# pvphan/camera-calibration

Hardware: AMD Instinct MI355X
Metric: LM iters/sec & residuals/sec, 10k-view checkerboard @1/2/4/8 GPU (higher is better)
Workload: dtype f64

## Files before the change

camera-calibration_amd/calibrate.py:

```python
import operator
import time

import numpy as np

from . import distortion
from . import engine
from . import fixed as fixedmod
from . import jacobian
from . import mathutils as mu
from . import uncertainty as uncertaintymod


class Calibrator:
    _λinitial = engine.LAMBDA_INITIAL
    _λmin = engine.LAMBDA_MIN
    _λmax = engine.LAMBDA_MAX
    _Pt_error_min = engine.PT_ERROR_MIN

    def __init__(self, distortionModel: distortion.DistortionModel, *, fixed=(), dtype="f64", device=0):
        self._distortionModel = distortionModel
        self.setFixed(fixed)
        self._jac = None
        self._dtype = dtype
        self._device = device
# ... 16 lines not shown
            return P0
        return fixedmod.applyFixedValues(P0, self._fixedValues)

    def calibrate(self, allDetections, maxIters):
        Ainitial, Winitial, kInitial = self.estimateCalibrationParameters(allDetections)
        return self.refineCalibrationParameters(Ainitial, Winitial, kInitial, allDetections,
                                                maxIters, shouldPrint=True)

    def calibrateExtended(self, allDetections, maxIters):
        sse, A, W, k = self.calibrate(allDetections, maxIters)
        return sse, A, W, k, self.uncertainty(A, W, k, allDetections)

    def uncertainty(self, A, W, k, allDetections):
        P = self._composeParameterVector(A, W, k).ravel()
        eng = self._resident.getFromDetections(allDetections)
        eng.setFixedShared(self._fixedMask)
        cov = eng.covariance(P, wantViews=True, wantCross=False)
        errs = eng.viewErrors(P)
        return uncertaintymod.fromEngineResults(self._distortionModel.sharedParameterNames(), cov, errs, eng.MN,
                                                values=P, fixedMask=self._fixedMask)

    def estimateCalibrationParameters(self, allDetections):
        from . import linearcalibrate
        offs, sensor, model = engine.packDetections(allDetections)
        A, W, k = linearcalibrate.estimateCalibrationParametersDevice(self._distortionModel, offs, sensor, model,
                                                                      self._device)
        return A, list(W), k

    def _refineHomographies(self, Hs, allDetections):
        offs, sensor, model = engine.packDetections(allDetections)
        return list(engine.refineHomographies(Hs, offs, sensor, model, 20, self._device))

    def _refineHomography(self, H, sensorPoints, modelPoints, jac=None):
        s = np.asarray(sensorPoints, dtype=np.float64).reshape(-1, 2)
        m = np.asarray(modelPoints, dtype=np.float64).reshape(-1, 3)
        offs = np.array([0, s.shape[0]], dtype=np.int64)
        return engine.refineHomographies(np.asarray(H, dtype=np.float64).reshape(1, 3, 3), offs, s, m, 20,
                                         self._device)[0]

    def _projectPointsHomography(self, H, modelPoints):
        modelPoints = np.asarray(modelPoints, dtype=np.float64)
        return mu.unhom((np.asarray(H, dtype=np.float64) @ mu.hom(modelPoints[:, :2]).T).T)

    def refineCalibrationParameters(self, Ainitial, Winitial, kInitial, allDetections,
                                    maxIters, shouldPrint=False):
        self._initializeJacobian()
        if not isinstance(self._jac, jacobian.ProjectionJacobian):
            raise TypeError(f"Calibrator._jac was replaced by {type(self._jac).__name__}: the device refinement "
                            "evaluates the closed-form projection Jacobian inside its kernels and cannot consult an "
                            "injected Jacobian object; use jacobian.ProjectionJacobian (or leave _jac unset)")
        maxIters = operator.index(maxIters)
        if maxIters <= 0:
            raise UnboundLocalError("local variable 'Pt_error' referenced before assignment")
        t0 = time.perf_counter()
        Pt = self._composeParameterVector(Ainitial, Winitial, kInitial)
        t1 = time.perf_counter()
        eng = self._resident.getFromDetections(allDetections)
        sse, P, iters, trace = self._refineOn(eng, Pt, maxIters, shouldPrint)
        t3 = time.perf_counter()
        Arefined, Wrefined, kRefined = self._decomposeParameterVector(P)
        self.lastSeconds.update(compose=t1 - t0, decompose=time.perf_counter() - t3)
        return sse, Arefined, Wrefined, kRefined

    def refinePacked(self, P0, viewOffsets, sensorPoints, modelPoints, maxIters, shouldPrint=False, sameProblem=False):
        if maxIters <= 0:
            raise UnboundLocalError("local variable 'Pt_error' referenced before assignment")
        eng = self._resident.get(viewOffsets, sensorPoints, modelPoints, sameProblem=sameProblem)
        return self._refineOn(eng, P0, maxIters, shouldPrint)

    def _refineOn(self, eng, P0, maxIters, shouldPrint):
        t0 = time.perf_counter()
        eng.setFixedShared(self._fixedMask)
        P0 = self._startPoint(P0)
        if not shouldPrint:
            out = eng.refine(P0, maxIters, self._λinitial, self._λmin, self._λmax, self._Pt_error_min)
        else:
            out = self._refineVerbose(eng, P0, maxIters)
        self.lastSeconds = dict(self._resident.lastSeconds, lm=time.perf_counter() - t0, iters=int(out[2]))
        self.lastTrace = out[3]
        return out

    def _refineVerbose(self, eng, P0, maxIters):
        ts = time.time()
        eng.lmBegin(P0, maxIters, self._λinitial, self._λmin, self._λmax, self._Pt_error_min)
        eng.lmRun(1)
        for it in range(maxIters):
            eng.lmRun(1)
            row, itersDone = eng.peekTrace(it)
            if itersDone > it:
                error = row[1] if not (row[2] < row[1]) else row[2]
                self._printIterationStats(it, ts, row[5:], error, row[3])
            if eng.lmDone():
                break
        return eng.lmEnd()

    def refinePoses(self, A, Winitial, k, allDetections, maxIters):
        modelId = self._distortionModel.modelId
        L = engine.NUM_SHARED[modelId]
        P = engine.composeParameters(modelId, A, Winitial, k, self._device)
        offs, sensor, model = engine.packDetections(allDetections)
        sse, poses, iters, status = engine.refinePoses(modelId, P[:L], P[L:].reshape(-1, 6), offs, sensor, model,
                                                       operator.index(maxIters), self._λinitial, self._λmin, self._λmax,
                                                       self._Pt_error_min, self._device)
        _, W, _ = engine.decomposeParameters(modelId, np.concatenate((P[:L], poses.ravel())), self._device)
        return sse, list(W), iters, status

    def estimatePoses(self, A, k, allDetections, maxIters=20):
        offs, sensor, model = engine.packDetections(allDetections)
        Hs = engine.estimateHomographies(offs, sensor, model, 20, self._device)
        Winitial = engine.computeExtrinsics(Hs, A, self._device)
        return self.refinePoses(A, Winitial, k, allDetections, maxIters)

    def _initializeJacobian(self):
        if self._jac is None:
            self._jac = jacobian.ProjectionJacobian(self._distortionModel, self._dtype, self._device)
# ... 34 lines not shown
```

camera-calibration_amd/csrc/calib_lm.hip:

```cpp
#include "../../include/calib_lm.h"
#include "kernels.hpp"
#include "host_rows.hpp"
#include "launch_plan.hpp"
#include "shard_layout.hpp"

#include <hip/hip_runtime.h>
#include <hip/hip_ext.h>
#include <algorithm>
#include <atomic>
#include <cmath>
#include <cstdio>
#include <cstdlib>
#include <dlfcn.h>
#include <chrono>
#include <future>
#include <memory>
#include <mutex>
#include <thread>
#include <cstring>
#include <new>
#include <string>
#include <type_traits>
#include <vector>

// ... 76 lines not shown
        return r.empty() ? "none" : r;
    }
    int model = 0, dtype = 0, device = 0;
    int L = 10, C = 16;
    hipStream_t own_stream = nullptr;
    hipStream_t stream = nullptr;

    bool has_problem = false;
    int64_t M = 0, MN = 0;
    int nv = 0;
    int n_items = 0;
    int64_t n_tiles = 0;
    int max_views_per_tile = 1;
    int uniform_n = 0;
    Knobs knobs;
    LaunchPlan plan;
    std::vector<ShardChunk> chunks;
    int64_t max_chunk_points = 0;
    DevBuf<unsigned char> uv, XY, Z, VC, J, r, y;
    template <typename U> static U* as(const DevBuf<unsigned char>& b) { return reinterpret_cast<U*>(b.p); }
    template <typename U> U* uv_as() const { return as<U>(uv); }
    template <typename U> U* XY_as() const { return as<U>(XY); }
    template <typename U> U* Z_as() const { return as<U>(Z); }
    template <typename U> U* VC_as() const { return as<U>(VC); }
    template <typename U> U* J_as() const { return as<U>(J); }
    template <typename U> U* r_as() const { return as<U>(r); }
    template <typename U> U* y_as() const { return as<U>(y); }
    DevBuf<int> pt_view, view_ext, item_n, view_item0, item_view;
    DevBuf<uint32_t> emit_tab;
    DevBuf<int32_t> stream_ops;
    int lm_mode = CALIB_LM_FUSED;
    uint32_t fixed_mask = 0;
    int num_cus = 256;
    DevBuf<int64_t> item_pt0;
    DevBuf<double> sse_part, G[2], bpart, part, red_own, P[2], Peval, trace;
    int n_bpart = 0;
    DevBuf<LMState> st, st_eval;
    double* red = nullptr;
    void* comm = nullptr;
    DevBuf<double> rccl_test;
    int comm_ranks = 0, comm_rank = 0;
    void* peer_mem = nullptr;
    std::vector<void*> peer_open;
    DevBuf<unsigned long long*> peer_slots;
    std::vector<unsigned long long*> peer_slot_host;
    DevBuf<int> peer_flags;
    int peer_world = 0, peer_rank = 0;
    unsigned peer_epoch = 0;
    double peer_timeout_s = 60.0;
    bool peer_connected = false;
    bool exchange_round = false;
    int* host_done = nullptr;
    int* host_done_dev = nullptr;
    bool lm_active = false;
    int lm_max_iters = 0;
    int rounds_enqueued = 0;

    bool cov_pending = false;
    std::vector<int64_t> ext_offsets;
    bool ext_offsets_on_device = false;
    DevBuf<int64_t> ext_offsets_dev;
    DevBuf<double> view_err, cov_css, cov_views, cov_cross;
    DevBuf<int> cov_flag;

    bool stage_ready = false;
    void* stage_pinned = nullptr;
    hipStream_t stage_stream[4] = {nullptr, nullptr, nullptr, nullptr};
    void* stage_buf[4][2] = {{nullptr, nullptr}, {nullptr, nullptr}, {nullptr, nullptr}, {nullptr, nullptr}};
    hipEvent_t stage_ev[4][2] = {{nullptr, nullptr}, {nullptr, nullptr}, {nullptr, nullptr}, {nullptr, nullptr}};

    bool prof = false;
    int prof_stride = 1;
    int64_t prof_seen[3] = {0, 0, 0};
    std::vector<hipEvent_t> ev;
    std::vector<int> ev_kind;
    size_t ev_used = 0;
};

namespace {

size_t tsize(const calib_handle_s* h) { return h->dtype == CALIB_DTYPE_F64 ? 8 : 4; }

int prof_reserve(calib_handle_s* h, int kind) {
    if (!h->prof || h->ev_used + 2 > h->ev.size()) return -1;
    if (h->prof_seen[kind]++ % h->prof_stride != 0) return -1;
    int idx = (int)h->ev_used;
    h->ev_used += 2;
    h->ev_kind[idx / 2] = kind;
    return idx;
}

template <typename F, typename... Args>
void launch_kind(calib_handle_s* h, int kind, F kernel, dim3 grid, dim3 block, size_t shmem, Args... args) {
    const int idx = prof_reserve(h, kind);
    if (idx >= 0)
        hipExtLaunchKernelGGL(kernel, grid, block, (uint32_t)shmem, h->stream, h->ev[(size_t)idx], h->ev[(size_t)idx + 1], 0, args...);
    else
        hipLaunchKernelGGL(kernel, grid, block, shmem, h->stream, args...);
}

calib_handle_s* const kNoHandle = nullptr;

static_assert(CALIB_MODEL_RADTAN == kRadtan && CALIB_MODEL_FISHEYE == kFisheye, "the C ABI's model ids are the kernels'");
template <int MODEL_, typename T_>
struct Form {
    static constexpr int MODEL = MODEL_, L = ModelTraits<MODEL_>::L, C = ModelTraits<MODEL_>::C;
// ... 396 lines not shown
        if (rc) return rc;
    }
    if (MN > 0) {
        const int rc = pack_points(h, lay, sensor_uv, model_xyz, lap);
        if (rc) return rc;
    }
    h->has_problem = true;
    return CALIB_OK;
}

struct LocalSlots { hipIpcMemHandle_t ipc; void* mem; int device; };
std::vector<LocalSlots> g_local_slots;
std::mutex g_local_slots_mutex;

void peer_release(calib_handle_s* h) {
    for (void* m : h->peer_open)
        if (m) (void)hipIpcCloseMemHandle(m);
    h->peer_open.clear();
    if (h->peer_mem) {
        std::lock_guard<std::mutex> lock(g_local_slots_mutex);
        for (size_t i = 0; i < g_local_slots.size(); ++i)
            if (g_local_slots[i].mem == h->peer_mem) { g_local_slots.erase(g_local_slots.begin() + (long)i); break; }
    }
    if (h->peer_mem) (void)hipFree(h->peer_mem);
    h->peer_mem = nullptr;
    h->peer_slots.release();
    h->peer_slot_host.clear();
    h->peer_flags.release();
    h->peer_connected = false;
    h->peer_world = 0;
}

int peer_fault_check(calib_handle_s* h) {
    if (!h->peer_connected) return CALIB_OK;
    int fault = 0;
    HIP_TRY(hipMemcpy(&fault, h->peer_flags.p, sizeof(int), hipMemcpyDeviceToHost));
    if (fault)
        return fail(CALIB_E_HIP, "peer exchange: a rank's contribution did not arrive before the deadline "
                                 "(the ranks no longer run in lockstep, or a peer died)");
    return CALIB_OK;
}

int lm_finish(calib_handle_s* h, LMState* s) {
    SYNC_H(h);
    HIP_TRY(hipMemcpy(s, st_cur(h), sizeof(*s), hipMemcpyDeviceToHost));
    h->lm_active = false;
    const int prc = peer_fault_check(h);
    if (prc) return prc;
    if (s->error == CALIB_E_SINGULAR)
        return fail(CALIB_E_SINGULAR, "Singular matrix: damped normal equations are not invertible");
    return CALIB_OK;
}

int lm_run(calib_handle_t h, int rounds, int check_every, bool sharded) {
    CHECK_H(h);
    if (!h->lm_active) return fail(CALIB_E_STATE, "calib_lm_begin has not been called");
    const bool peers = sharded && h->peer_connected;
    for (int i = 0; i < rounds; ++i) {
        h->exchange_round = peers;
        int rc = calib_lm_local(h);
        h->exchange_round = false;
        if (rc) return rc;
        if (sharded && !peers) {
            rc = calib_lm_allreduce(h);
            if (rc) return rc;
        }
        rc = calib_lm_update(h);
        if (rc) return rc;
        if (peers && h->host_done && *static_cast<volatile int*>(h->host_done) == 2)
            return fail(CALIB_E_HIP, "peer exchange: a rank's contribution did not arrive before the deadline "
                                     "(the ranks no longer run in lockstep, or a peer died); no further rounds are enqueued");
        if (check_every > 0 && !sharded && h->host_done) {
            if (*static_cast<volatile int*>(h->host_done)) break;
        } else if (check_every > 0 && (i + 1) % check_every == 0 && i + 1 < rounds) {
            int done = 0;
            rc = calib_lm_done(h, &done);
            if (rc) return rc;
            if (done) break;
        }
    }
    return CALIB_OK;
}

int check_views(int64_t num_views, const int64_t* view_offsets, const double* sensor_uv, const double* model_xyz) {
    if (num_views < 0 || !view_offsets) return fail(CALIB_E_INVALID, "null argument");
    if (num_views == 0) return CALIB_OK;
    const int64_t MN = view_offsets[num_views];
    if (view_offsets[0] != 0 || MN < 0 || (MN > 0 && (!sensor_uv || !model_xyz)))
        return fail(CALIB_E_INVALID, "bad view_offsets / point arrays");
    for (int64_t i = 0; i < num_views; ++i)
        if (view_offsets[i + 1] < view_offsets[i]) return fail(CALIB_E_INVALID, "view_offsets must be non-decreasing");
    return CALIB_OK;
}

int use_device(int device_id) {
    int ndev = 0;
    HIP_TRY(hipGetDeviceCount(&ndev));
    if (device_id < 0 || device_id >= ndev) return fail(CALIB_E_HIP, "no such HIP device (no CPU fallback)");
    HIP_TRY(hipSetDevice(device_id));
    return CALIB_OK;
}

int homography_pipeline(int64_t num_views, const int64_t* view_offsets, const double* sensor_uv,
                        const double* model_xyz, double* H, bool dlt, int refine_iters, int device_id) {
    if (!H) return fail(CALIB_E_INVALID, "null argument");
    int rc = check_views(num_views, view_offsets, sensor_uv, model_xyz);
    if (rc || num_views == 0) return rc;
    rc = use_device(device_id);
    if (rc) return rc;
    const int64_t MN = view_offsets[num_views];
    std::vector<double> xy((size_t)MN * 2);
    for (int64_t p = 0; p < MN; ++p) { xy[2 * p] = model_xyz[3 * p]; xy[2 * p + 1] = model_xyz[3 * p + 1]; }
    DevBuf<int64_t> doffs;
    DevBuf<double2> duv, dxy;
    DevBuf<double> dH;
    HIP_TRY(doffs.alloc((size_t)num_views + 1));
    HIP_TRY(duv.alloc((size_t)std::max<int64_t>(MN, 1)));
    HIP_TRY(dxy.alloc((size_t)std::max<int64_t>(MN, 1)));
    HIP_TRY(dH.alloc((size_t)num_views * 9));
    HIP_TRY(hipMemcpy(doffs.p, view_offsets, ((size_t)num_views + 1) * 8, hipMemcpyHostToDevice));
    if (MN) HIP_TRY(hipMemcpy(duv.p, sensor_uv, (size_t)MN * 16, hipMemcpyHostToDevice));
    if (MN) HIP_TRY(hipMemcpy(dxy.p, xy.data(), (size_t)MN * 16, hipMemcpyHostToDevice));
    if (!dlt) HIP_TRY(hipMemcpy(dH.p, H, (size_t)num_views * 72, hipMemcpyHostToDevice));
    const unsigned blocks = (unsigned)((num_views + 15) / 16);
    if (dlt) {
        hipLaunchKernelGGL(dlt_kernel, dim3(blocks), dim3(256), 0, 0, doffs.p, (const double2*)duv.p, (const double2*)dxy.p,
                           num_views, dH.p);
// ... 233 lines not shown

    auto fetch2 = [&](const void* dev, double* out) -> int {
        if (h->dtype == CALIB_DTYPE_F64) {
            HIP_TRY(hipMemcpy(out, dev, (size_t)MN * 16, hipMemcpyDeviceToHost));
        } else {
            std::vector<float> tmp((size_t)MN * 2);
            HIP_TRY(hipMemcpy(tmp.data(), dev, tmp.size() * 4, hipMemcpyDeviceToHost));
            for (size_t i = 0; i < tmp.size(); ++i) out[i] = tmp[i];
        }
        return CALIB_OK;
    };
    if (out_y && MN) { rc = fetch2(h->y.p, out_y); if (rc) return rc; }
    if (out_r && MN) { rc = fetch2(h->r.p, out_r); if (rc) return rc; }
    if (out_Jc && MN) {
        const int C = h->C;
        const size_t cnt = MN4 * C * 2;
        std::vector<double> tmp(cnt);
        if (h->dtype == CALIB_DTYPE_F64) {
            HIP_TRY(hipMemcpy(tmp.data(), h->J.p, cnt * 8, hipMemcpyDeviceToHost));
        } else {
            std::vector<float> tf(cnt);
            HIP_TRY(hipMemcpy(tf.data(), h->J.p, cnt * 4, hipMemcpyDeviceToHost));
            for (size_t i = 0; i < cnt; ++i) tmp[i] = tf[i];
        }
        for (int64_t p = 0; p < MN; ++p)
            for (int c = 0; c < C; ++c) {
                out_Jc[(p * 2 + 0) * C + c] = tmp[(size_t)jIndex(p, c, C) * 2 + 0];
                out_Jc[(p * 2 + 1) * C + c] = tmp[(size_t)jIndex(p, c, C) * 2 + 1];
            }
    }
    return CALIB_OK;
}

int calib_lm_reduce_size(calib_handle_t h, int64_t* out_num_doubles) {
    if (!h || !out_num_doubles) return fail(CALIB_E_INVALID, "null argument");
    *out_num_doubles = reduceSize(h->L);
    return CALIB_OK;
}

int calib_lm_bind_reduce_buffer(calib_handle_t h, void* reduce_dev) {
    CHECK_H(h);
    SYNC_H(h);
    HIP_TRY(h->red_own.alloc((size_t)reduceSize(h->L)));
    h->red = reduce_dev ? reinterpret_cast<double*>(reduce_dev) : h->red_own.p;
    return CALIB_OK;
}

int calib_lm_begin(calib_handle_t h, const double* P0, int max_iters, double lam_init, double lam_min,
                   double lam_max, double err_min) {
    CHECK_H(h);
    int rc = need_problem(h);
    if (rc) return rc;
    if (!P0) return fail(CALIB_E_INVALID, "P0 is null");
    h->cov_pending = false;
    if (max_iters <= 0)
        return fail(CALIB_E_INVALID, "max_iters must be >= 1 (the reference raises UnboundLocalError "
                                     "for maxIters=0, src/calibrate.py:171)");
    if (h->nv != h->M)
        return fail(CALIB_E_SINGULAR, "a view without points makes J^T J + lambda diag(J^T J) singular");
    const size_t ts = tsize(h);
    const int64_t K = numParams(h);
    if (h->lm_mode == CALIB_LM_TWO_KERNEL)
        HIP_TRY(h->J.alloc((size_t)((h->max_chunk_points + 3) / 4 * 4) * h->C * 2 * ts));
    for (int b = 0; b < 2; ++b) {
        const bool fresh = !h->G[b].p || h->G[b].n < (size_t)num_records(h) * kGStride;
        HIP_TRY(h->G[b].alloc((size_t)num_records(h) * kGStride));
        if (fresh) HIP_TRY(hipMemsetAsync(h->G[b].p, 0, h->G[b].n * 8, h->stream));
    }
    HIP_TRY(h->bpart.alloc(((size_t)std::max(h->n_items, 1) + h->chunks.size()) * kPartStride));
    HIP_TRY(h->part.alloc((size_t)2 * h->plan.schur_blocks * variantSize(h->L)));
    HIP_TRY(h->red_own.alloc((size_t)reduceSize(h->L)));
    if (!h->red) h->red = h->red_own.p;
    HIP_TRY(h->P[0].alloc((size_t)K));
    HIP_TRY(h->P[1].alloc((size_t)K));
    HIP_TRY(h->st.alloc(2));
    HIP_TRY(h->trace.alloc((size_t)max_iters * (CALIB_TRACE_HEADER + h->L)));
    HIP_TRY(hipMemsetAsync(h->trace.p, 0, (size_t)max_iters * (CALIB_TRACE_HEADER + h->L) * 8, h->stream));
    HIP_TRY(hipMemcpyAsync(h->P[0].p, P0, (size_t)K * 8, hipMemcpyHostToDevice, h->stream));
    HIP_TRY(hipMemcpyAsync(h->P[1].p, P0, (size_t)K * 8, hipMemcpyHostToDevice, h->stream));
    LMState s;
    std::memset(&s, 0, sizeof(s));
    s.lam = lam_init; s.lam_min = lam_min; s.lam_max = lam_max; s.err_min = err_min;
    if (!h->host_done) {
        void* p = nullptr;
        if (hipHostMalloc(&p, sizeof(int), hipHostMallocMapped) == hipSuccess) h->host_done = static_cast<int*>(p);
        else (void)hipGetLastError();
        void* dp = nullptr;
        if (h->host_done && hipHostGetDevicePointer(&dp, h->host_done, 0) == hipSuccess) h->host_done_dev = static_cast<int*>(dp);
        else (void)hipGetLastError();
    }
    if (h->host_done) {
        if (h->lm_active) SYNC_H(h);
        *h->host_done = 0;
        s.notify = h->host_done_dev;
    }
    s.cur = 1;
    s.fixed_mask = (int)h->fixed_mask;
    s.max_iters = max_iters;
    HIP_TRY(hipMemsetAsync(h->st.p, 0, 2 * sizeof(LMState), h->stream));
    HIP_TRY(hipMemcpyAsync(h->st.p, &s, sizeof(s), hipMemcpyHostToDevice, h->stream));
    SYNC_H(h);
    h->lm_active = true;
    h->lm_max_iters = max_iters;
    h->rounds_enqueued = 0;
    return CALIB_OK;
}

int calib_lm_local(calib_handle_t h) {
    CHECK_H(h);
    if (!h->lm_active) return fail(CALIB_E_STATE, "calib_lm_begin has not been called");
    LMState* st = st_cur(h);
    int rc = CALIB_OK;
    if (h->rounds_enqueued == 0) {
        rc = launch_view_setup(h, h->P[0].p, h->P[1].p, st, 1);
        if (rc) return rc;
    }
    if (h->lm_mode == CALIB_LM_FUSED) {
        rc = launch_fused(h, st, 1);
        if (rc) return rc;
        return launch_schur_reduce(h, st, h->red);
    }
    h->n_bpart = 0;
    for (const auto& c : h->chunks) {
        rc = launch_jacobian(h, h->P[0].p, h->P[1].p, st, 1, true, true, false, false, c.p0, c.p1);
        if (rc) return rc;
        rc = launch_gram(h, st, 1, c.item0, c.item1, c.p0);
        if (rc) return rc;
    }
    return launch_schur_reduce(h, st, h->red);
}

int calib_lm_update(calib_handle_t h) {
    CHECK_H(h);
    if (!h->lm_active) return fail(CALIB_E_STATE, "calib_lm_begin has not been called");
    const int rc = launch_update_backsub(h);
    h->rounds_enqueued += 1;
    return rc;
}

int calib_lm_done(calib_handle_t h, int* out_done) {
    CHECK_H(h);
    if (!h->lm_active || !out_done) return fail(CALIB_E_STATE, "no LM run active");
    LMState s;
    HIP_TRY(hipMemcpyAsync(&s, st_cur(h), sizeof(s), hipMemcpyDeviceToHost, h->stream));
    SYNC_H(h);
    *out_done = s.done;
    return peer_fault_check(h);
}

int calib_lm_peek_trace(calib_handle_t h, int iter, double* out_row, int* out_iters) {
    CHECK_H(h);
    if (!h->lm_active || !out_row || !out_iters) return fail(CALIB_E_STATE, "no LM run active");
    if (iter < 0 || iter >= h->lm_max_iters) return fail(CALIB_E_INVALID, "trace row out of range");
    LMState s;
    const size_t w = (size_t)(CALIB_TRACE_HEADER + h->L);
    HIP_TRY(hipMemcpyAsync(&s, st_cur(h), sizeof(s), hipMemcpyDeviceToHost, h->stream));
    HIP_TRY(hipMemcpyAsync(out_row, h->trace.p + (size_t)iter * w, w * 8, hipMemcpyDeviceToHost, h->stream));
    SYNC_H(h);
// ... 516 lines not shown
    return CALIB_OK;
}

int calib_compose_params(int model, int64_t num_views, const double* A, const double* W, const double* k,
                         double* P_out, int device_id) {
    if (!known_model(model)) return fail(CALIB_E_INVALID, "unknown distortion model");
    if (num_views < 0 || !A || !k || !P_out || (num_views > 0 && !W)) return fail(CALIB_E_INVALID, "null argument");
    const int nk = num_distortion(model), L = 5 + nk;
    P_out[0] = A[0]; P_out[1] = A[4]; P_out[2] = A[1]; P_out[3] = A[2]; P_out[4] = A[5];
    for (int j = 0; j < nk; ++j) P_out[5 + j] = k[j];
    if (num_views == 0) return CALIB_OK;
    int rc = use_device(device_id);
    if (rc) return rc;
    DevBuf<double> dW, dP;
    HIP_TRY(dW.alloc((size_t)num_views * 16));
    HIP_TRY(dP.alloc((size_t)L + 6 * (size_t)num_views));
    HIP_TRY(hipMemcpy(dW.p, W, (size_t)num_views * 128, hipMemcpyHostToDevice));
    hipLaunchKernelGGL(compose_views_kernel, dim3((unsigned)((num_views + 255) / 256)), dim3(256), 0, 0, dW.p, num_views, L, dP.p);
    LAUNCHED(kNoHandle, "compose_views_kernel");
    HIP_TRY(hipMemcpy(P_out + L, dP.p + L, (size_t)num_views * 48, hipMemcpyDeviceToHost));
    return CALIB_OK;
}

int calib_decompose_params(int model, int64_t num_views, const double* P, double* A_out, double* W_out,
                           double* k_out, int device_id) {
    if (!known_model(model)) return fail(CALIB_E_INVALID, "unknown distortion model");
    if (num_views < 0 || !P || (num_views > 0 && !W_out)) return fail(CALIB_E_INVALID, "null argument");
    const int nk = num_distortion(model), L = 5 + nk;
    if (A_out) {
        const double a[9] = {P[0], P[2], P[3], 0.0, P[1], P[4], 0.0, 0.0, 1.0};
        std::memcpy(A_out, a, sizeof(a));
    }
    if (k_out) for (int j = 0; j < nk; ++j) k_out[j] = P[5 + j];
    if (num_views == 0) return CALIB_OK;
    int rc = use_device(device_id);
    if (rc) return rc;
    DevBuf<double> dW, dP;
    HIP_TRY(dW.alloc((size_t)num_views * 16));
    HIP_TRY(dP.alloc((size_t)L + 6 * (size_t)num_views));
    HIP_TRY(hipMemcpy(dP.p, P, ((size_t)L + 6 * (size_t)num_views) * 8, hipMemcpyHostToDevice));
    hipLaunchKernelGGL(decompose_views_kernel, dim3((unsigned)((num_views + 255) / 256)), dim3(256), 0, 0, dP.p, num_views, L, dW.p);
    LAUNCHED(kNoHandle, "decompose_views_kernel");
    HIP_TRY(hipMemcpy(W_out, dW.p, (size_t)num_views * 128, hipMemcpyDeviceToHost));
    return CALIB_OK;
}

int calib_refine_awk(calib_handle_t h, double* A_inout, double* W_inout, double* k_inout, int max_iters,
                     double lam_init, double lam_min, double lam_max, double err_min, double* out_sse,
                     int* out_iters, double* out_trace) {
    CHECK_H(h);
    int rc = need_problem(h);
    if (rc) return rc;
    if (!A_inout || !k_inout || (h->M > 0 && !W_inout)) return fail(CALIB_E_INVALID, "null argument");
    std::vector<double> P((size_t)numParams(h));
    rc = calib_compose_params(h->model, h->M, A_inout, W_inout, k_inout, P.data(), h->device);
    if (rc) return rc;
    rc = calib_refine(h, P.data(), max_iters, lam_init, lam_min, lam_max, err_min, out_sse, out_iters, out_trace);
    if (rc) return rc;
    return calib_decompose_params(h->model, h->M, P.data(), A_inout, W_inout, k_inout, h->device);
}

int calib_profile_enable(calib_handle_t h, int on) {
    CHECK_H(h);
    SYNC_H(h);
    if (on && h->ev.empty()) {
        h->ev.resize(kEventPool);
        h->ev_kind.assign(kEventPool / 2, 0);
        for (auto& e : h->ev) HIP_TRY(hipEventCreate(&e));
    }
    h->prof = on != 0;
    h->prof_stride = on > 1 ? on : 1;
    h->prof_seen[0] = h->prof_seen[1] = h->prof_seen[2] = 0;
    h->ev_used = 0;
    return CALIB_OK;
}

int calib_profile_read(calib_handle_t h, int which, double* out_total_ms, int64_t* out_launches) {
    CHECK_H(h);
    if (!out_total_ms || !out_launches) return fail(CALIB_E_INVALID, "null argument");
    SYNC_H(h);
    double total = 0.0;
    int64_t count = 0;
    for (size_t i = 0; i + 1 < h->ev_used; i += 2) {
        if (h->ev_kind[i / 2] != which) continue;
        float ms = 0.f;
        HIP_TRY(hipEventElapsedTime(&ms, h->ev[i], h->ev[i + 1]));
        total += ms;
        count += 1;
    }
    *out_total_ms = total;
    *out_launches = count;
    return CALIB_OK;
}

int calib_view_errors(calib_handle_t h, const double* P, double* out_view_sse, double* out_view_rms,
                      double* out_view_max) {
    CHECK_H(h);
    int rc = need_problem(h);
    if (rc) return rc;
    if (!P) return fail(CALIB_E_INVALID, "P is null");
    if (h->lm_active)
        return fail(CALIB_E_STATE, "a stepping LM run is active on this handle (calib_lm_end it first)");
    const int64_t M = h->M;
    if (M == 0) return CALIB_OK;
    if (!h->ext_offsets_on_device) {
        HIP_TRY(h->ext_offsets_dev.alloc((size_t)M + 1));
        HIP_TRY(hipMemcpy(h->ext_offsets_dev.p, h->ext_offsets.data(), ((size_t)M + 1) * 8, hipMemcpyHostToDevice));
        h->ext_offsets_on_device = true;
    }
    HIP_TRY(h->view_err.alloc((size_t)M * 3));
    HIP_TRY(hipMemcpyAsync(h->Peval.p, P, (size_t)numParams(h) * 8, hipMemcpyHostToDevice, h->stream));
    rc = launch_view_setup(h, h->Peval.p, nullptr, h->st_eval.p, 0);
// ... 108 lines not shown
```

camera-calibration_amd/csrc/kernels.hpp:

```cpp
#pragma once
#include "point_model.hpp"
#include <stdint.h>
#include <type_traits>

namespace calib {

constexpr int kTile = 256;
constexpr int kGramChunk = 512;
constexpr int kGramUnroll = 4;
constexpr int kGRows = 0;
constexpr int kGStride = 96;
__host__ __device__ __forceinline__ constexpr int gvSlot(int L, int j) { return j < 5 ? L + 1 + j : 16 + L + 2; }
__host__ __device__ __forceinline__ constexpr int gvOfSlot(int L, int slot) {
    const int m = slot >> 4, n = (slot & 15) - L;
    return (m == 0 && n >= 1 && n <= 5) ? n - 1 : ((m == 1 && n == 2) ? 5 : -1);
}
constexpr int kPartStride = 112;
constexpr int kMaxL = 10;

constexpr int kEmitZero = 256;
constexpr int kEmitTile = 264;
constexpr int kEmitTabSize = kGStride + kPartStride;
inline void buildEmitTable(int C, uint32_t* tab ) {
    const int L = C - 6;
// ... 1490 lines not shown
    const double gci = useB ? gS : gA;
#pragma unroll
    for (int j = 0; j < L; ++j) {
        brow[j] = useB ? bS[j] : bA[j];
        row[j] = brow[j] - (useB ? sB[j] : sA[j]);
    }
    row[L] = gci - (useB ? rhsB : rhsA);
#pragma unroll
    for (int j = 0; j < L; ++j) if (j == i) row[j] += lam * brow[j];
    const int fixed_mask = in->fixed_mask;
    const bool fixed_i = (fixed_mask >> i) & 1;
    if (fixed_mask != 0) {
#pragma unroll
        for (int j = 0; j < L; ++j) {
            const bool fixed_j = (fixed_mask >> j) & 1;
            row[j] = (fixed_i || fixed_j) ? (j == i ? 1.0 : 0.0) : row[j];
        }
        row[L] = fixed_i ? 0.0 : row[L];
    }
    if (!done) {
        double saved[L + 1];
#pragma unroll
        for (int j = 0; j <= L; ++j) saved[j] = row[j];
        if (!spd_solve_wave0<L>(row, i, dc)) {
            int myCol = -1;
            double d = 0.0;
            if (gauss_jordan16<L, true>(saved, i, myCol, d)) { error = -3; done = true; }
#pragma unroll
            for (int c = 0; c < L; ++c) dc[c] = group_sum16(myCol == c ? d : 0.0);
        }
    } else {
#pragma unroll
        for (int c = 0; c < L; ++c) dc[c] = 0.0;
    }

    if (writer) {
        if (i < L) {
#pragma unroll
            for (int j = 0; j < L; ++j) out->B[i * L + j] = brow[j];
            out->gc[i] = gci;
            double dci = 0.0;
#pragma unroll
            for (int c = 0; c < L; ++c) if (c == i) dci = dc[c];
            out->dc[i] = dci;
            if (!done) Pb[cur ^ 1][i] = fixed_i ? Pb[cur][i] : Pb[cur][i] + dci;
        }
        if (w0) {
            out->lam = lam; out->err_cur = err_cur_new; out->last_err = last_err;
            out->lam_min = in->lam_min; out->lam_max = in->lam_max; out->err_min = in->err_min;
            out->cur = cur; out->round = round + 1; out->iters = iters; out->max_iters = in->max_iters;
            out->done = done ? 1 : 0; out->error = error; out->accepted_last = accepted; out->fixed_mask = fixed_mask;
            out->notify = in->notify;
            if (done && in->notify) __hip_atomic_store(in->notify, 1, __ATOMIC_RELAXED, __HIP_MEMORY_SCOPE_SYSTEM);
        }
    }
    cur_out = cur;
    lam_out = lam;
    return !done;
}

template <int L, typename T>
__device__ __forceinline__ void finish_view(const double (&V)[21], const double (&invd)[6], const double (&z)[6],
                                            double coef, int c, int v, const int* __restrict__ view_ext,
                                            const double* __restrict__ Pc, double* __restrict__ Pn,
                                            T* __restrict__ VC) {
    double w[6];
#pragma unroll
    for (int m = 0; m < 6; ++m) w[m] = group_sum16(coef * z[m]);
    double d[6];
    backward6(V, invd, w, d);
    const int64_t o = L + 6 * (int64_t)view_ext[v];
    double en[6];
#pragma unroll
    for (int m = 0; m < 6; ++m) en[m] = Pc[o + m] + d[m];
    if (c < 6) {
        double ev = en[0];
#pragma unroll
        for (int m = 1; m < 6; ++m) ev = (c == m) ? en[m] : ev;
        Pn[o + c] = ev;
    }
    const double deg = 0.017453292519943295;
    double sn[3], cs[3];
    {
        const int a = c & 3;
        const double th = (a == 1 ? en[1] : (a == 2 ? en[2] : en[0])) * deg;
        double s1, c1;
        sincos(th, &s1, &c1);
        if (fabs(th) <= 1e-8) { s1 = 0.0; c1 = 1.0; }
        sn[0] = quad_bcast<0>(s1); sn[1] = quad_bcast<1>(s1); sn[2] = quad_bcast<2>(s1);
        cs[0] = quad_bcast<0>(c1); cs[1] = quad_bcast<1>(c1); cs[2] = quad_bcast<2>(c1);
    }
    const double sx = sn[0], cx = cs[0], sy = sn[1], cy = cs[1], sz = sn[2], cz = cs[2];
    const double o18[18] = {cz * cy, cz * sy * sx - sz * cx, cz * sy * cx + sz * sx,
                            sz * cy, sz * sy * sx + cz * cx, sz * sy * cx - cz * sx,
                            -sy, cy * sx, cy * cx, en[3], en[4], en[5],
                            deg * cz * cy, deg * sz * cy, -deg * sy, -deg * sz, deg * cz, 0.0};
    double mine = o18[0];
#pragma unroll
    for (int j = 1; j < 16; ++j) mine = (c == j) ? o18[j] : mine;
    T* dst = VC + (int64_t)v * kViewStride;
    dst[c] = (T)mine;
    if (c < 2) dst[16 + c] = (T)(c == 0 ? o18[16] : o18[17]);
}

template <typename T>
struct UpdArgs {
// ... 781 lines not shown
```

camera-calibration_amd/csrc/launch_plan.hpp:

```cpp
#pragma once
#include "../../include/calib_lm.h"
#include "kernels.hpp"

#include <algorithm>
#include <cstdint>
#include <cstdlib>
#include <cstring>

namespace calib {

constexpr int kUpdSmallViews = 4096;
constexpr int kUpdLaneViews = 24576;
constexpr int kWideHeadViews = 4096;

struct Knobs {
    int lm_mode = CALIB_LM_FUSED;
    int head_loads = 0;
    int items_per_wave = 0;
    int upd_lane_views = kUpdLaneViews;
    int upd_small_views = kUpdSmallViews;
    int gram_form = 0;
    int stream_mode = -1;
    int stream_waves = 0;
    int gram_wpi = 0;
    int64_t chunk_points = (int64_t)1 << 26;
    bool timing = false;
};

inline Knobs readKnobs() {
    Knobs k;
    if (const char* e = std::getenv("CALIB_LM_MODE")) k.lm_mode = std::atoi(e) ? CALIB_LM_TWO_KERNEL : CALIB_LM_FUSED;
    if (const char* e = std::getenv("CALIB_HEAD_LOADS")) k.head_loads = std::strcmp(e, "narrow") == 0 ? 1 : (std::strcmp(e, "wide") == 0 ? 2 : 0);
    if (const char* e = std::getenv("CALIB_ITEMS_PER_WAVE")) k.items_per_wave = std::max(0, std::min(16, std::atoi(e)));
    if (const char* e = std::getenv("CALIB_UPD_LANE_VIEWS")) k.upd_lane_views = std::max(1, std::atoi(e));
    if (const char* e = std::getenv("CALIB_UPD_SMALL_VIEWS")) k.upd_small_views = std::max(0, std::atoi(e));
    if (const char* e = std::getenv("CALIB_GRAM_FORM")) k.gram_form = std::strcmp(e, "tile") == 0 ? 1 : (std::strcmp(e, "block") == 0 ? 2 : 0);
    if (const char* e = std::getenv("CALIB_FUSED_STREAM")) k.stream_mode = std::atoi(e) > 0 ? 1 : (std::atoi(e) == 0 ? 0 : -1);
    if (const char* e = std::getenv("CALIB_STREAM_WAVES")) k.stream_waves = std::max(0, std::atoi(e));
    if (const char* e = std::getenv("CALIB_GRAM_WPI")) {
        const int w = std::atoi(e);
        if (w == 1 || w == 2 || w == 4) k.gram_wpi = w;
    }
    if (const char* e = std::getenv("CALIB_CHUNK_POINTS")) k.chunk_points = std::max<int64_t>(1, std::atoll(e));
    k.timing = std::getenv("CALIB_TIMING") != nullptr;
    return k;
}

struct ShardShape {
    int nv = 0, n_items = 0, uniform_n = 0;
    int64_t MN = 0;
};

enum class FusedForm {
    TwoKernel,
    Tile,
    TileMulti,
    Block44,
    Stream,
};
enum class UpdateForm {
    Small,
    Lane,
    Wide16,
};

struct LaunchPlan {
    FusedForm fused = FusedForm::Tile;
    int fused_wpi = 1;
    int ipw = 1;
    int fused_blocks = 0;
    int gram_wpi = 1;
    int stream_share = 0;
    int stream_waves = 0;
    bool wide_heads = false;
    UpdateForm update = UpdateForm::Small;
    int schur_blocks = 1;
    int update_blocks = 1;
    bool stream() const { return stream_share > 0; }
};

inline LaunchPlan makePlan(const ShardShape& s, int dtype, int lm_mode, const Knobs& k, int num_cus) {
    LaunchPlan p;
    const double avg = s.n_items ? (double)s.MN / s.n_items : 0.0;
    p.gram_wpi = avg >= 128 ? 4 : (avg >= 64 ? 2 : 1);
    p.fused_wpi = s.n_items >= 2048 ? 1 : p.gram_wpi;
    if (k.gram_wpi > 0) p.gram_wpi = p.fused_wpi = k.gram_wpi;

    const int un = s.uniform_n;
    const bool can = dtype == CALIB_DTYPE_F64 && un >= 64 && (un & 3) == 0 && s.MN < ((int64_t)1 << 31) && s.nv >= 1;
    if (lm_mode == CALIB_LM_FUSED && can && k.stream_mode != 0) {
        const int slots = k.stream_waves > 0 ? k.stream_waves : kFusedWaves * kStreamMinBlocks * num_cus;
        const int waves = std::max(1, std::min(slots, s.nv));
        if (k.stream_mode == 1 || s.nv >= 2 * slots) {
            const int64_t groups = (int64_t)s.nv * (un / 4);
            p.stream_share = (int)((groups + waves - 1) / waves);
            p.stream_waves = (int)((groups + p.stream_share - 1) / p.stream_share);
// ... 39 lines not shown
```

camera-calibration_amd/engine.py:

```python
import ctypes

import numpy as np

from . import _native as nat
from . import fixed as fixedmod

LAMBDA_INITIAL = 1e-3
LAMBDA_MIN = 1e-10
LAMBDA_MAX = 1e+10
PT_ERROR_MIN = 1e-12

MODEL_IDS = {"radtan": nat.MODEL_RADTAN, "fisheye": nat.MODEL_FISHEYE}
NUM_SHARED = {nat.MODEL_RADTAN: 10, nat.MODEL_FISHEYE: 9}
DTYPE_IDS = {"f64": nat.DTYPE_F64, "fp64": nat.DTYPE_F64, "float64": nat.DTYPE_F64,
             "f32": nat.DTYPE_F32, "fp32": nat.DTYPE_F32, "float32": nat.DTYPE_F32}


def _stack(arrays, width):
    M = len(arrays)
    if M == 0:
        return np.zeros(0, dtype=np.int64), np.empty((0, width))
    fast = True
    for a in arrays:
        if type(a) is not np.ndarray or a.dtype != np.float64 or a.ndim != 2 or a.shape[1] != width:
# ... 164 lines not shown
        return share.value, waves.value

    def _P(self, P):
        P = np.ascontiguousarray(np.asarray(P, dtype=np.float64).ravel())
        if P.shape[0] != self.K:
            raise ValueError(f"Expected shape ({self.K},), got {P.shape}")
        return P

    def evaluate(self, P, wantY=False, wantR=False, wantJ=False):
        P = self._P(P)
        y = np.empty((self.MN, 2)) if wantY else None
        r = np.empty((self.MN, 2)) if wantR else None
        Jc = np.empty((self.MN, 2, self.C)) if wantJ else None
        sse = ctypes.c_double(0.0)
        nat.check(self._lib.calib_eval(self._h, nat.dptr(P), nat.dptr(y), nat.dptr(r), nat.dptr(Jc),
                                       ctypes.byref(sse)))
        return {"y": y, "r": r, "Jc": Jc, "sse": sse.value}

    def normalEquations(self, P):
        P = self._P(P)
        B = np.empty((self.L, self.L))
        E = np.empty((self.M, self.L, 6))
        V = np.empty((self.M, 6, 6))
        g = np.empty(self.K)
        nat.check(self._lib.calib_normal_eq(self._h, nat.dptr(P), nat.dptr(B), nat.dptr(E), nat.dptr(V),
                                            nat.dptr(g)))
        return B, E, V, g

    def stepDelta(self, P, lam):
        P = self._P(P)
        d = np.empty(self.K)
        nat.check(self._lib.calib_lm_step_delta(self._h, nat.dptr(P), float(lam), nat.dptr(d)))
        return d

    def refine(self, P0, maxIters, lamInit=LAMBDA_INITIAL, lamMin=LAMBDA_MIN, lamMax=LAMBDA_MAX,
               errMin=PT_ERROR_MIN):
        P = self._P(P0).copy()
        if int(maxIters) <= 0:
            raise UnboundLocalError("local variable 'Pt_error' referenced before assignment "
                                    "(maxIters=0, src/calibrate.py:171)")
        trace = np.zeros((int(maxIters), nat.TRACE_HEADER + self.L))
        sse = ctypes.c_double(0.0)
        iters = ctypes.c_int(0)
        nat.check(self._lib.calib_refine(self._h, nat.dptr(P), int(maxIters), float(lamInit), float(lamMin),
                                         float(lamMax), float(errMin), ctypes.byref(sse),
                                         ctypes.byref(iters), nat.dptr(trace)))
        return sse.value, P, iters.value, trace[:iters.value]

    def refineAWk(self, A, W, k, maxIters, lamInit=LAMBDA_INITIAL, lamMin=LAMBDA_MIN, lamMax=LAMBDA_MAX,
                  errMin=PT_ERROR_MIN):
        if int(maxIters) <= 0:
            raise UnboundLocalError("local variable 'Pt_error' referenced before assignment "
                                    "(maxIters=0, src/calibrate.py:171)")
        A = np.ascontiguousarray(A, dtype=np.float64).reshape(3, 3).copy()
        W = np.ascontiguousarray(np.asarray(W, dtype=np.float64).reshape(-1, 4, 4)).copy()
        k = np.ascontiguousarray(k, dtype=np.float64).ravel().copy()
        if W.shape[0] != self.M or k.shape[0] != self.L - 5:
            raise ValueError(f"Expected {self.M} poses and {self.L - 5} distortion coefficients, "
                             f"got {W.shape[0]} and {k.shape[0]}")
        trace = np.zeros((int(maxIters), nat.TRACE_HEADER + self.L))
        sse = ctypes.c_double(0.0)
        iters = ctypes.c_int(0)
        nat.check(self._lib.calib_refine_awk(self._h, nat.dptr(A), nat.dptr(W), nat.dptr(k), int(maxIters),
                                             float(lamInit), float(lamMin), float(lamMax), float(errMin),
                                             ctypes.byref(sse), ctypes.byref(iters), nat.dptr(trace)))
        return sse.value, A, W, k, iters.value, trace[:iters.value]

    def lmBegin(self, P0, maxIters, lamInit=LAMBDA_INITIAL, lamMin=LAMBDA_MIN, lamMax=LAMBDA_MAX,
                errMin=PT_ERROR_MIN):
        P = self._P(P0)
        self._lmMaxIters = int(maxIters)
        nat.check(self._lib.calib_lm_begin(self._h, nat.dptr(P), int(maxIters), float(lamInit),
                                           float(lamMin), float(lamMax), float(errMin)))

    def reduceSize(self):
        n = ctypes.c_int64(0)
        nat.check(self._lib.calib_lm_reduce_size(self._h, ctypes.byref(n)))
        return n.value

    def bindReduceBuffer(self, devicePointer):
        nat.check(self._lib.calib_lm_bind_reduce_buffer(self._h, ctypes.c_void_p(devicePointer or 0)))

    def lmLocal(self):
        nat.check(self._lib.calib_lm_local(self._h))

    def lmUpdate(self):
        nat.check(self._lib.calib_lm_update(self._h))

    def lmRun(self, rounds, checkEvery=0):
        nat.check(self._lib.calib_lm_run(self._h, int(rounds), int(checkEvery)))

    def lmRunSharded(self, rounds, checkEvery=0):
        nat.check(self._lib.calib_lm_run_sharded(self._h, int(rounds), int(checkEvery)))

    def peerPrepare(self, nranks, rank):
        buf = (ctypes.c_ubyte * 64)()
        nat.check(self._lib.calib_peer_prepare(self._h, int(nranks), int(rank), ctypes.cast(buf, ctypes.c_void_p)))
        return bytes(buf)

    def peerConnect(self, handles, timeoutSeconds=60.0):
        blob = b"".join(handles)
        buf = (ctypes.c_ubyte * len(blob)).from_buffer_copy(blob)
        nat.check(self._lib.calib_peer_connect(self._h, ctypes.cast(buf, ctypes.c_void_p), float(timeoutSeconds)))

    def peerSelfTest(self, rounds=64, timeoutSeconds=10.0):
        nat.check(self._lib.calib_peer_selftest(self._h, int(rounds), float(timeoutSeconds)))

    def peerShutdown(self):
        nat.check(self._lib.calib_peer_shutdown(self._h))
# ... 301 lines not shown
```

Measured before the change: 30.54 billion.

## Bound in-flight LM rounds with a run-ahead window and compose poses on device

Adds a windowed launcher that caps how many LM rounds are enqueued ahead of the device, using a device-written round counter in mapped host memory. The goal is to stop enqueuing long runs of wasted rounds after convergence while keeping the launch queue full. Calibrator.refineCalibrationParameters now goes through refineAWk, which uploads the poses and composes and decomposes the parameter vector with GPU kernels, replacing host-side compose and decompose. This adds host spin-polling and a new code path that could stall if the window is too small.

```diff
diff --git a/camera-calibration_amd/calibrate.py b/camera-calibration_amd/calibrate.py
--- a/camera-calibration_amd/calibrate.py
+++ b/camera-calibration_amd/calibrate.py
@@ -92,6 +92,8 @@
         maxIters = operator.index(maxIters)
         if maxIters <= 0:
             raise UnboundLocalError("local variable 'Pt_error' referenced before assignment")
+        if not shouldPrint:
+            return self._refineAWk(Ainitial, Winitial, kInitial, allDetections, maxIters)
         t0 = time.perf_counter()
         Pt = self._composeParameterVector(Ainitial, Winitial, kInitial)
         t1 = time.perf_counter()
@@ -101,6 +103,23 @@
         Arefined, Wrefined, kRefined = self._decomposeParameterVector(P)
         self.lastSeconds.update(compose=t1 - t0, decompose=time.perf_counter() - t3)
         return sse, Arefined, Wrefined, kRefined
+
+    def _refineAWk(self, A, W, k, allDetections, maxIters):
+        eng = self._resident.getFromDetections(allDetections)
+        t0 = time.perf_counter()
+        eng.setFixedShared(self._fixedMask)
+        if self._fixedValues:
+            A = np.asarray(A, dtype=np.float64).reshape(3, 3)
+            k = np.asarray(k, dtype=np.float64).ravel()
+            sh = self._startPoint(np.concatenate(([A[0, 0], A[1, 1], A[0, 1], A[0, 2], A[1, 2]], k)))
+            A = np.array([[sh[0], sh[2], sh[3]], [0.0, sh[1], sh[4]], [0.0, 0.0, 1.0]])
+            k = sh[5:]
+        sse, Arefined, Wrefined, kRefined, iters, trace = eng.refineAWk(A, W, k, maxIters, self._λinitial, self._λmin,
+                                                                        self._λmax, self._Pt_error_min)
+        self.lastSeconds = dict(self._resident.lastSeconds, lm=time.perf_counter() - t0, iters=int(iters),
+                                compose=0.0, decompose=0.0)
+        self.lastTrace = trace
+        return sse, Arefined, list(Wrefined), kRefined
 
     def refinePacked(self, P0, viewOffsets, sensorPoints, modelPoints, maxIters, shouldPrint=False, sameProblem=False):
         if maxIters <= 0:
diff --git a/camera-calibration_amd/csrc/calib_lm.hip b/camera-calibration_amd/csrc/calib_lm.hip
--- a/camera-calibration_amd/csrc/calib_lm.hip
+++ b/camera-calibration_amd/csrc/calib_lm.hip
@@ -152,6 +152,7 @@
     bool exchange_round = false;
     int* host_done = nullptr;
     int* host_done_dev = nullptr;
+    DevBuf<double> awk_W;
     bool lm_active = false;
     int lm_max_iters = 0;
     int rounds_enqueued = 0;
@@ -654,9 +655,105 @@
     return CALIB_OK;
 }
 
+int lm_prepare(calib_handle_s* h, int max_iters) {
+    h->cov_pending = false;
+    if (max_iters <= 0)
+        return fail(CALIB_E_INVALID, "max_iters must be >= 1 (the reference raises UnboundLocalError "
+                                     "for maxIters=0, src/calibrate.py:171)");
+    if (h->nv != h->M)
+        return fail(CALIB_E_SINGULAR, "a view without points makes J^T J + lambda diag(J^T J) singular");
+    const size_t ts = tsize(h);
+    const int64_t K = numParams(h);
+    if (h->lm_mode == CALIB_LM_TWO_KERNEL)
+        HIP_TRY(h->J.alloc((size_t)((h->max_chunk_points + 3) / 4 * 4) * h->C * 2 * ts));
+    for (int b = 0; b < 2; ++b) {
+        const bool fresh = !h->G[b].p || h->G[b].n < (size_t)num_records(h) * kGStride;
+        HIP_TRY(h->G[b].alloc((size_t)num_records(h) * kGStride));
+        if (fresh) HIP_TRY(hipMemsetAsync(h->G[b].p, 0, h->G[b].n * 8, h->stream));
+    }
+    HIP_TRY(h->bpart.alloc(((size_t)std::max(h->n_items, 1) + h->chunks.size()) * kPartStride));
+    HIP_TRY(h->part.alloc((size_t)2 * h->plan.schur_blocks * variantSize(h->L)));
+    HIP_TRY(h->red_own.alloc((size_t)reduceSize(h->L)));
+    if (!h->red) h->red = h->red_own.p;
+    HIP_TRY(h->P[0].alloc((size_t)K));
+    HIP_TRY(h->P[1].alloc((size_t)K));
+    HIP_TRY(h->st.alloc(2));
+    HIP_TRY(h->trace.alloc((size_t)max_iters * (CALIB_TRACE_HEADER + h->L)));
+    HIP_TRY(hipMemsetAsync(h->trace.p, 0, (size_t)max_iters * (CALIB_TRACE_HEADER + h->L) * 8, h->stream));
+    return CALIB_OK;
+}
+
+int lm_start(calib_handle_s* h, int max_iters, double lam_init, double lam_min, double lam_max, double err_min) {
+    LMState s;
+    std::memset(&s, 0, sizeof(s));
+    s.lam = lam_init; s.lam_min = lam_min; s.lam_max = lam_max; s.err_min = err_min;
+    if (!h->host_done) {
+        void* p = nullptr;
+        if (hipHostMalloc(&p, 2 * sizeof(int), hipHostMallocMapped) == hipSuccess) h->host_done = static_cast<int*>(p);
+        else (void)hipGetLastError();
+        void* dp = nullptr;
+        if (h->host_done && hipHostGetDevicePointer(&dp, h->host_done, 0) == hipSuccess) h->host_done_dev = static_cast<int*>(dp);
+        else (void)hipGetLastError();
+    }
+    if (h->host_done) {
+        if (h->lm_active) SYNC_H(h);
+        h->host_done[0] = 0;
+        h->host_done[1] = 0;
+        s.notify = h->host_done_dev;
+    }
+    s.cur = 1;
+    s.fixed_mask = (int)h->fixed_mask;
+    s.max_iters = max_iters;
+    HIP_TRY(hipMemsetAsync(h->st.p, 0, 2 * sizeof(LMState), h->stream));
+    HIP_TRY(hipMemcpyAsync(h->st.p, &s, sizeof(s), hipMemcpyHostToDevice, h->stream));
+    SYNC_H(h);
+    h->lm_active = true;
+    h->lm_max_iters = max_iters;
+    h->rounds_enqueued = 0;
+    return CALIB_OK;
+}
+
+int lm_run_windowed(calib_handle_s* h, int rounds) {
+    volatile int* word = h->host_done;
+    const int window = h->knobs.run_ahead;
+    const int target = h->rounds_enqueued + rounds;
+    int lost = 0;
+    for (;;) {
+        const bool done = word[0] != 0;
+        const int finished = word[1];
+        int n = runAheadQuota(target, h->rounds_enqueued, std::max(finished, lost), done, window);
+        if (n == 0) {
+            if (done || h->rounds_enqueued >= target) return CALIB_OK;
+            const int seen = word[1];
+            const auto deadline = std::chrono::steady_clock::now() + std::chrono::seconds(2);
+            while (word[1] == seen && word[0] == 0) {
+                if (std::chrono::steady_clock::now() > deadline) {
+                    const hipError_t e = hipStreamQuery(h->stream);
+                    if (e != hipSuccess && e != hipErrorNotReady)
+                        return fail(CALIB_E_HIP, std::string("hipStreamQuery: ") + hipGetErrorString(e) +
+                                                 " (kernels enqueued since the last successful synchronisation: " + h->recentKernels() + ")");
+                    SYNC_H(h);
+                    lost = h->rounds_enqueued;
+                    break;
+                }
+                std::this_thread::yield();
+            }
+            continue;
+        }
+        for (; n > 0; --n) {
+            int rc = calib_lm_local(h);
+            if (rc) return rc;
+            rc = calib_lm_update(h);
+            if (rc) return rc;
+            if (word[0]) return CALIB_OK;
+        }
+    }
+}
+
 int lm_run(calib_handle_t h, int rounds, int check_every, bool sharded) {
     CHECK_H(h);
     if (!h->lm_active) return fail(CALIB_E_STATE, "calib_lm_begin has not been called");
+    if (check_every > 0 && !sharded && h->host_done) return lm_run_windowed(h, rounds);
     const bool peers = sharded && h->peer_connected;
     for (int i = 0; i < rounds; ++i) {
         h->exchange_round = peers;
@@ -672,9 +769,7 @@
         if (peers && h->host_done && *static_cast<volatile int*>(h->host_done) == 2)
             return fail(CALIB_E_HIP, "peer exchange: a rank's contribution did not arrive before the deadline "
                                      "(the ranks no longer run in lockstep, or a peer died); no further rounds are enqueued");
-        if (check_every > 0 && !sharded && h->host_done) {
-            if (*static_cast<volatile int*>(h->host_done)) break;
-        } else if (check_every > 0 && (i + 1) % check_every == 0 && i + 1 < rounds) {
+        if (check_every > 0 && (i + 1) % check_every == 0 && i + 1 < rounds) {
             int done = 0;
             rc = calib_lm_done(h, &done);
             if (rc) return rc;
@@ -1014,58 +1109,12 @@
     int rc = need_problem(h);
     if (rc) return rc;
     if (!P0) return fail(CALIB_E_INVALID, "P0 is null");
-    h->cov_pending = false;
-    if (max_iters <= 0)
-        return fail(CALIB_E_INVALID, "max_iters must be >= 1 (the reference raises UnboundLocalError "
-                                     "for maxIters=0, src/calibrate.py:171)");
-    if (h->nv != h->M)
-        return fail(CALIB_E_SINGULAR, "a view without points makes J^T J + lambda diag(J^T J) singular");
-    const size_t ts = tsize(h);
+    rc = lm_prepare(h, max_iters);
+    if (rc) return rc;
     const int64_t K = numParams(h);
-    if (h->lm_mode == CALIB_LM_TWO_KERNEL)
-        HIP_TRY(h->J.alloc((size_t)((h->max_chunk_points + 3) / 4 * 4) * h->C * 2 * ts));
-    for (int b = 0; b < 2; ++b) {
-        const bool fresh = !h->G[b].p || h->G[b].n < (size_t)num_records(h) * kGStride;
-        HIP_TRY(h->G[b].alloc((size_t)num_records(h) * kGStride));
-        if (fresh) HIP_TRY(hipMemsetAsync(h->G[b].p, 0, h->G[b].n * 8, h->stream));
-    }
-    HIP_TRY(h->bpart.alloc(((size_t)std::max(h->n_items, 1) + h->chunks.size()) * kPartStride));
-    HIP_TRY(h->part.alloc((size_t)2 * h->plan.schur_blocks * variantSize(h->L)));
-    HIP_TRY(h->red_own.alloc((size_t)reduceSize(h->L)));
-    if (!h->red) h->red = h->red_own.p;
-    HIP_TRY(h->P[0].alloc((size_t)K));
-    HIP_TRY(h->P[1].alloc((size_t)K));
-    HIP_TRY(h->st.alloc(2));
-    HIP_TRY(h->trace.alloc((size_t)max_iters * (CALIB_TRACE_HEADER + h->L)));
-    HIP_TRY(hipMemsetAsync(h->trace.p, 0, (size_t)max_iters * (CALIB_TRACE_HEADER + h->L) * 8, h->stream));
     HIP_TRY(hipMemcpyAsync(h->P[0].p, P0, (size_t)K * 8, hipMemcpyHostToDevice, h->stream));
     HIP_TRY(hipMemcpyAsync(h->P[1].p, P0, (size_t)K * 8, hipMemcpyHostToDevice, h->stream));
-    LMState s;
-    std::memset(&s, 0, sizeof(s));
-    s.lam = lam_init; s.lam_min = lam_min; s.lam_max = lam_max; s.err_min = err_min;
-    if (!h->host_done) {
-        void* p = nullptr;
-        if (hipHostMalloc(&p, sizeof(int), hipHostMallocMapped) == hipSuccess) h->host_done = static_cast<int*>(p);
-        else (void)hipGetLastError();
-        void* dp = nullptr;
-        if (h->host_done && hipHostGetDevicePointer(&dp, h->host_done, 0) == hipSuccess) h->host_done_dev = static_cast<int*>(dp);
-        else (void)hipGetLastError();
-    }
-    if (h->host_done) {
-        if (h->lm_active) SYNC_H(h);
-        *h->host_done = 0;
-        s.notify = h->host_done_dev;
-    }
-    s.cur = 1;
-    s.fixed_mask = (int)h->fixed_mask;
-    s.max_iters = max_iters;
-    HIP_TRY(hipMemsetAsync(h->st.p, 0, 2 * sizeof(LMState), h->stream));
-    HIP_TRY(hipMemcpyAsync(h->st.p, &s, sizeof(s), hipMemcpyHostToDevice, h->stream));
-    SYNC_H(h);
-    h->lm_active = true;
-    h->lm_max_iters = max_iters;
-    h->rounds_enqueued = 0;
-    return CALIB_OK;
+    return lm_start(h, max_iters, lam_init, lam_min, lam_max, err_min);
 }
 
 int calib_lm_local(calib_handle_t h) {
@@ -1688,12 +1737,48 @@
     int rc = need_problem(h);
     if (rc) return rc;
     if (!A_inout || !k_inout || (h->M > 0 && !W_inout)) return fail(CALIB_E_INVALID, "null argument");
-    std::vector<double> P((size_t)numParams(h));
-    rc = calib_compose_params(h->model, h->M, A_inout, W_inout, k_inout, P.data(), h->device);
-    if (rc) return rc;
-    rc = calib_refine(h, P.data(), max_iters, lam_init, lam_min, lam_max, err_min, out_sse, out_iters, out_trace);
-    if (rc) return rc;
-    return calib_decompose_params(h->model, h->M, P.data(), A_inout, W_inout, k_inout, h->device);
+    rc = lm_prepare(h, max_iters);
+    if (rc) return rc;
+    const int64_t M = h->M, K = numParams(h);
+    const int L = h->L, nk = L - 5;
+    const unsigned blocks = (unsigned)((M + 255) / 256);
+    double shared[kMaxL] = {A_inout[0], A_inout[4], A_inout[1], A_inout[2], A_inout[5]};
+    for (int j = 0; j < nk; ++j) shared[5 + j] = k_inout[j];
+    HIP_TRY(hipMemcpyAsync(h->P[0].p, shared, (size_t)L * 8, hipMemcpyHostToDevice, h->stream));
+    if (M > 0) {
+        HIP_TRY(h->awk_W.alloc((size_t)M * 16));
+        HostRows w;
+        w.flat = W_inout; w.width = 16;
+        rc = upload_staged(h, h->awk_W.p, w, (size_t)M * 128);
+        if (rc) return rc;
+        hipLaunchKernelGGL(compose_views_kernel, dim3(blocks), dim3(256), 0, h->stream, (const double*)h->awk_W.p, M, L, h->P[0].p);
+        LAUNCHED(h, "compose_views_kernel");
+    }
+    HIP_TRY(hipMemcpyAsync(h->P[1].p, h->P[0].p, (size_t)K * 8, hipMemcpyDeviceToDevice, h->stream));
+    rc = lm_start(h, max_iters, lam_init, lam_min, lam_max, err_min);
+    if (rc) return rc;
+    rc = calib_lm_run(h, max_iters + 1, 8);
+    if (rc) return rc;
+    LMState s;
+    rc = lm_finish(h, &s);
+    if (rc) return rc;
+    const double* P = h->P[s.round == 0 ? 0 : s.cur].p;
+    if (M > 0) {
+        hipLaunchKernelGGL(decompose_views_kernel, dim3(blocks), dim3(256), 0, h->stream, P, M, L, h->awk_W.p);
+        LAUNCHED(h, "decompose_views_kernel");
+        HIP_TRY(hipMemcpyAsync(W_inout, h->awk_W.p, (size_t)M * 128, hipMemcpyDeviceToHost, h->stream));
+    }
+    HIP_TRY(hipMemcpyAsync(shared, P, (size_t)L * 8, hipMemcpyDeviceToHost, h->stream));
+    if (out_trace && s.iters > 0)
+        HIP_TRY(hipMemcpyAsync(out_trace, h->trace.p, (size_t)s.iters * (CALIB_TRACE_HEADER + L) * 8, hipMemcpyDeviceToHost,
+                               h->stream));
+    SYNC_H(h);
+    const double a[9] = {shared[0], shared[2], shared[3], 0.0, shared[1], shared[4], 0.0, 0.0, 1.0};
+    std::memcpy(A_inout, a, sizeof(a));
+    for (int j = 0; j < nk; ++j) k_inout[j] = shared[5 + j];
+    if (out_sse) *out_sse = s.last_err;
+    if (out_iters) *out_iters = s.iters;
+    return CALIB_OK;
 }
 
 int calib_profile_enable(calib_handle_t h, int on) {
diff --git a/camera-calibration_amd/csrc/kernels.hpp b/camera-calibration_amd/csrc/kernels.hpp
--- a/camera-calibration_amd/csrc/kernels.hpp
+++ b/camera-calibration_amd/csrc/kernels.hpp
@@ -1566,6 +1566,7 @@
             out->done = done ? 1 : 0; out->error = error; out->accepted_last = accepted; out->fixed_mask = fixed_mask;
             out->notify = in->notify;
             if (done && in->notify) __hip_atomic_store(in->notify, 1, __ATOMIC_RELAXED, __HIP_MEMORY_SCOPE_SYSTEM);
+            if (in->notify) in->notify[1] = round + 1;
         }
     }
     cur_out = cur;
diff --git a/camera-calibration_amd/csrc/launch_plan.hpp b/camera-calibration_amd/csrc/launch_plan.hpp
--- a/camera-calibration_amd/csrc/launch_plan.hpp
+++ b/camera-calibration_amd/csrc/launch_plan.hpp
@@ -1,6 +1,7 @@
 #pragma once
 #include "../../include/calib_lm.h"
 #include "kernels.hpp"
+#include "run_ahead.hpp"
 
 #include <algorithm>
 #include <cstdint>
@@ -24,6 +25,7 @@
     int stream_waves = 0;
     int gram_wpi = 0;
     int64_t chunk_points = (int64_t)1 << 26;
+    int run_ahead = kRunAheadDefault;
     bool timing = false;
 };
 
@@ -42,6 +44,7 @@
         if (w == 1 || w == 2 || w == 4) k.gram_wpi = w;
     }
     if (const char* e = std::getenv("CALIB_CHUNK_POINTS")) k.chunk_points = std::max<int64_t>(1, std::atoll(e));
+    if (const char* e = std::getenv("CALIB_RUN_AHEAD")) k.run_ahead = std::atoi(e) == 0 ? 0 : std::max(1, std::atoi(e));
     k.timing = std::getenv("CALIB_TIMING") != nullptr;
     return k;
 }
diff --git a/camera-calibration_amd/csrc/run_ahead.hpp b/camera-calibration_amd/csrc/run_ahead.hpp
--- /dev/null
+++ b/camera-calibration_amd/csrc/run_ahead.hpp
@@ -0,0 +1,18 @@
+#pragma once
+
+namespace calib {
+
+constexpr int kRunAheadDefault = 4;
+
+inline int runAheadQuota(int requested, int enqueued, int finished, bool done, int window) {
+    if (done || enqueued >= requested) return 0;
+    const int left = requested - enqueued;
+    if (window <= 0) return left;
+    if (finished > enqueued) finished = enqueued;
+    if (finished < 0) finished = 0;
+    const int room = window - (enqueued - finished);
+    if (room <= 0) return 0;
+    return room < left ? room : left;
+}
+
+}
diff --git a/camera-calibration_amd/engine.py b/camera-calibration_amd/engine.py
--- a/camera-calibration_amd/engine.py
+++ b/camera-calibration_amd/engine.py
@@ -240,9 +240,9 @@
         if int(maxIters) <= 0:
             raise UnboundLocalError("local variable 'Pt_error' referenced before assignment "
                                     "(maxIters=0, src/calibrate.py:171)")
-        A = np.ascontiguousarray(A, dtype=np.float64).reshape(3, 3).copy()
-        W = np.ascontiguousarray(np.asarray(W, dtype=np.float64).reshape(-1, 4, 4)).copy()
-        k = np.ascontiguousarray(k, dtype=np.float64).ravel().copy()
+        A = np.array(A, dtype=np.float64, order="C").reshape(3, 3)
+        W = np.array(W, dtype=np.float64, order="C").reshape(-1, 4, 4)
+        k = np.array(k, dtype=np.float64, order="C").ravel()
         if W.shape[0] != self.M or k.shape[0] != self.L - 5:
             raise ValueError(f"Expected {self.M} poses and {self.L - 5} distortion coefficients, "
                              f"got {W.shape[0]} and {k.shape[0]}")
```

New measurement: 30.52 billion. About the same (-0.0%).
